# acappemin/Video-to-Audio-and-Piano-RP

Hardware: AMD Instinct MI355X
Metric: mel-frames/sec (10s VGGSound shape, 32-step CFM, CFG 2.0) (higher is better)
Workload: dtype bf16x3; 1 GPU; BASELINE.json configs[1]: 1 clip(s)/GPU x 750 latent frames x 128 ch, 32-point sway grid = 31 CFG evaluations (62 DiT forwards), T5 context 16 tokens, V2A zero roll; clips_per_gpu=1, global_clips=1, parallelism=clip-sharded x1, 1 all-gather, hipgraph=True, schedule=three streams, side_streams=True, cascade_passes=1

## Files before the change

### video-to-audio-and-piano-rp_amd/csrc/gemm_8phase.hip

```cpp
#include "gemm_common.h"

namespace {

#if defined(V2A_GEMM_PROBE) && defined(V2A_8PH_SKIP)
constexpr int kSkip = V2A_8PH_SKIP;
#else
constexpr int kSkip = 0;
#endif

template <int EPI, typename OutT, int MODE>
__global__ __launch_bounds__(512) void gemm_bf16_8ph_kernel(GemmParams p) {
  constexpr bool STAGGER = MODE != 2;
  constexpr int BM = 256, BN = 256, WM = 128, WN = 64, TM = 8, TN = 4;
  constexpr int HALF = 128 * 128;
  constexpr int BUF = 4 * HALF;
  static_assert(EPI != V2A_EPI_GEGLU || (TN % 2 == 0), "GEGLU needs value/gate tile pairs");
  extern __shared__ __attribute__((aligned(16))) char smem_raw[];

  const int tid = threadIdx.x;
  const int lane = tid & 63;
  const int wave = __builtin_amdgcn_readfirstlane(tid >> 6);
  const int wr = wave >> 2, wc = wave & 3;
  const int lr = lane & 15, lq = lane >> 4;

  int tm, tn;
  tile_of_block(p, blockIdx.x, tm, tn);
  const int m0 = tm * BM, n0 = tn * BN;

  f32x4 acc[TM][TN];
#pragma unroll
  for (int i = 0; i < TM; ++i)
#pragma unroll
    for (int j = 0; j < TN; ++j) acc[i][j] = f32x4{0.f, 0.f, 0.f, 0.f};

  const int srow = lane >> 3;
  const uint32_t schunk_b = (uint32_t)(((lane & 7) ^ srow) << 4);
  uint32_t woff[2][2];
#pragma unroll
  for (int s = 0; s < 2; ++s)
#pragma unroll
    for (int i = 0; i < 2; ++i) {
      const int r = 8 * (wave + 8 * i) + srow;
      const int wrw = n0 + 64 * (r >> 5) + (r & 31) + 32 * s;
      woff[s][i] = (uint32_t)(((int64_t)(wrw < p.N ? wrw : p.N - 1) * p.ldw) * 2) + schunk_b;
    }
  const char* wbase = reinterpret_cast<const char*>(p.w);
  const int nk = p.K / 64;

  const int nseg = p.nseg;
  const int64_t a0 = (int64_t)p.a[0];
  const int64_t da1 = nseg > 1 ? (int64_t)p.a[1] - a0 : 0, da2 = nseg > 2 ? (int64_t)p.a[2] - (int64_t)p.a[1] : 0;
  const int32_t ldb0 = (int32_t)(p.lda[0] * 2);
  const int32_t dl1 = nseg > 1 ? (int32_t)(p.lda[1] * 2) - ldb0 : 0, dl2 = nseg > 2 ? (int32_t)((p.lda[2] - p.lda[1]) * 2) : 0;
  const int kend0 = nseg > 1 ? p.kend[0] : 0x7fffffff, kend1 = nseg > 2 ? p.kend[1] : 0x7fffffff;
  const int dk2 = nseg > 2 ? p.kend[1] - p.kend[0] : 0;
  const int kl = p.s3_kl;
  const int nkl = kl > 0 ? kl / 64 : 0x3fffffff;
  const int klog = kl > 0 ? kl : p.K;
  const int sb0 = kl > 0 ? (int)(2 * p.alo[0]) : 0;
  const int dsb1 = kl > 0 && nseg > 1 ? (int)(2 * p.alo[1]) - sb0 : 0;
  const int dsb2 = kl > 0 && nseg > 2 ? (int)(2 * p.alo[2]) - (sb0 + dsb1) : 0;
  const int64_t wlo = (int64_t)kl * 2;
  const char* aptr[2];
  int aleft[2] = {0, 0};
  uint32_t aoff[2][2];
  auto a_setup = [&](int s, int kt) {
    const bool p1 = kt >= nkl, p2 = kt >= 2 * nkl;
    const int k0 = (kt - (p1 ? nkl : 0) - (p2 ? nkl : 0)) * 64;
    const bool s1 = k0 >= kend0, s2 = k0 >= kend1;
    const int kbeg = (s1 ? kend0 : 0) + (s2 ? dk2 : 0);
    const int lo = p2 ? sb0 + (s1 ? dsb1 : 0) + (s2 ? dsb2 : 0) : 0;
    aptr[s] = reinterpret_cast<const char*>(a0 + (s1 ? da1 : 0) + (s2 ? da2 : 0)) + (int64_t)(k0 - kbeg) * 2 + lo;
    const uint32_t ldb = (uint32_t)(ldb0 + (s1 ? dl1 : 0) + (s2 ? dl2 : 0));
    const int kstop = min(klog, s2 ? 0x7fffffff : (s1 ? kend1 : kend0));
    aleft[s] = (kstop - k0) >> 6;
#pragma unroll
    for (int i = 0; i < 2; ++i) {
      const int r = 8 * (wave + 8 * i) + srow;
      const int ar = m0 + r + ((r >= 64) ? 64 : 0) + 64 * s;
      aoff[s][i] = (uint32_t)(ar < p.M ? ar : p.M - 1) * ldb + schunk_b;
    }
  };
  auto stage_a = [&](int s, int kt, int buf) {
    if (aleft[s] == 0) a_setup(s, kt);
    char* dst = smem_raw + buf * BUF + s * HALF;
#pragma unroll
    for (int i = 0; i < 2; ++i)
      __builtin_amdgcn_global_load_lds((const __attribute__((address_space(1))) void*)(aptr[s] + aoff[s][i]),
                                       (__attribute__((address_space(3))) void*)(dst + (wave + 8 * i) * 1024), 16, 0, 0);
    aptr[s] += 128;
    --aleft[s];
  };
  const char* wptr = wbase;
  int wleft = 0;
  auto stage_b = [&](int kt, int buf) {
    if (wleft == 0) {
      const bool p1 = kt >= nkl, p2 = kt >= 2 * nkl;
      const int ktl = kt - (p1 ? nkl : 0) - (p2 ? nkl : 0);
      wptr = wbase + (int64_t)ktl * 128 + (p1 && !p2 ? wlo : 0);
      wleft = min(nkl, nk) - ktl;
    }
#pragma unroll
    for (int s = 0; s < 2; ++s) {
      char* dst = smem_raw + buf * BUF + (2 + s) * HALF;
#pragma unroll
      for (int i = 0; i < 2; ++i) {
        uint32_t wo = woff[s][i];
        asm volatile("" : "+v"(wo));
        __builtin_amdgcn_global_load_lds((const __attribute__((address_space(1))) void*)(wptr + wo),
                                         (__attribute__((address_space(3))) void*)(dst + (wave + 8 * i) * 1024), 16, 0, 0);
      }
    }
    wptr += 128;
    --wleft;
  };

  const int a_frag_off = (64 * wr + lr) * 128;
  const int b_frag_off = (32 * wc + lr) * 128;
  const int ch0 = ((0 + lq) ^ (lr & 7)) << 4, ch1 = ((4 + lq) ^ (lr & 7)) << 4;
  bf16x8 af[4][2], bf0[2][2], bf1[2][2];
  auto read_a = [&](int s, int buf) {
    const char* base = smem_raw + buf * BUF + s * HALF + a_frag_off;
#pragma unroll
    for (int i = 0; i < 4; ++i) {
      af[i][0] = *reinterpret_cast<const bf16x8*>(base + i * 2048 + ch0);
      af[i][1] = *reinterpret_cast<const bf16x8*>(base + i * 2048 + ch1);
    }
  };
  auto read_b = [&](int s, int buf, bf16x8 (&bf)[2][2]) {
    const char* base = smem_raw + buf * BUF + (2 + s) * HALF + b_frag_off;
#pragma unroll
    for (int j = 0; j < 2; ++j) {
      bf[j][0] = *reinterpret_cast<const bf16x8*>(base + j * 2048 + ch0);
      bf[j][1] = *reinterpret_cast<const bf16x8*>(base + j * 2048 + ch1);
    }
  };
  const int rows_valid = (p.dbg & 512) ? 256 : p.M - m0;
  const bool need0 = wr * 128 < rows_valid, need1 = wr * 128 + 64 < rows_valid;
  auto quadrant = [&](auto sa_c, auto sb_c, const bf16x8 (&bf)[2][2]) {
    constexpr int SA = decltype(sa_c)::value, SB = decltype(sb_c)::value;
    if (!(SA == 0 ? need0 : need1)) return;
    __builtin_amdgcn_s_setprio(1);
#pragma unroll
    for (int kk = 0; kk < 2; ++kk)
#pragma unroll
      for (int i = 0; i < 4; ++i)
#pragma unroll
        for (int j = 0; j < 2; ++j)
          acc[4 * SA + i][2 * SB + j] = __builtin_amdgcn_mfma_f32_16x16x32_bf16(af[i][kk], bf[j][kk], acc[4 * SA + i][2 * SB + j], 0, 0, 0);
    __builtin_amdgcn_s_setprio(0);
  };
  using I0 = std::integral_constant<int, 0>;
  using I1 = std::integral_constant<int, 1>;

  float* rs_lds = reinterpret_cast<float*>(smem_raw + 2 * BUF);
  const bool scaled = p.rssq != nullptr && p.vec_epi;
  RowScaleLoad rsl;
  if (scaled && tid < 256) rowscale_load(p, m0 + tid, rsl);
  stage_a(0, 0, 0);
  stage_b(0, 0);
  stage_a(1, 0, 0);
  if (nk > 1) {
    stage_a(0, 1, 1);
    stage_b(1, 1);
    if (scaled && tid < 256) rs_lds[tid] = rowscale_finish(p, rsl);
    asm volatile("s_waitcnt vmcnt(6)" ::: "memory");
  } else {
    if (scaled && tid < 256) rs_lds[tid] = rowscale_finish(p, rsl);
    asm volatile("s_waitcnt vmcnt(0)" ::: "memory");
  }
  __builtin_amdgcn_s_barrier();
  if constexpr (STAGGER) {
    if (wr == 1) __builtin_amdgcn_s_barrier();
  }

  auto ktile = [&](auto buf_c, int t) {
    constexpr int B = decltype(buf_c)::value;
    if (!(kSkip & 4) || t == 0) read_a(0, B);
    if (!(kSkip & 1) || t == 0) read_b(0, B, bf0);
    __builtin_amdgcn_sched_barrier(0);
    __builtin_amdgcn_s_barrier();
    quadrant(I0{}, I0{}, bf0);
    __builtin_amdgcn_sched_barrier(0);
    __builtin_amdgcn_s_barrier();
    if (!(kSkip & 1) || t == 0) read_b(1, B, bf1);
    if (t + 1 < nk && !(kSkip & 8)) stage_a(1, t + 1, B ^ 1);
    __builtin_amdgcn_sched_barrier(0);
    __builtin_amdgcn_s_barrier();
    quadrant(I0{}, I1{}, bf1);
    __builtin_amdgcn_sched_barrier(0);
    __builtin_amdgcn_s_barrier();
    if (!(kSkip & 4) || t == 0) read_a(1, B);
    if (t + 2 < nk && !(kSkip & 8)) stage_a(0, t + 2, B);
    __builtin_amdgcn_sched_barrier(0);
    __builtin_amdgcn_s_barrier();
    quadrant(I1{}, I1{}, bf1);
    __builtin_amdgcn_sched_barrier(0);
    __builtin_amdgcn_s_barrier();
    if (t + 2 < nk) {
      if (!(kSkip & 2)) stage_b(t + 2, B);
      asm volatile("s_waitcnt vmcnt(6)" ::: "memory");
    } else {
      asm volatile("s_waitcnt vmcnt(0)" ::: "memory");
    }
    __builtin_amdgcn_sched_barrier(0);
    __builtin_amdgcn_s_barrier();
    quadrant(I1{}, I0{}, bf0);
    __builtin_amdgcn_sched_barrier(0);
    __builtin_amdgcn_s_barrier();
  };
  for (int t = 0; t < nk; t += 2) {
    ktile(I0{}, t);
    if (t + 1 < nk) ktile(I1{}, t + 1);
  }
  if constexpr (STAGGER) {
    if (wr == 0) __builtin_amdgcn_s_barrier();
  }
  if (p.vec_epi) {
    static_assert(8 * 16 * (WN + 4) * 4 <= 2 * BUF, "epilogue slabs must fit in the ring memory");
    float* tile = reinterpret_cast<float*>(smem_raw) + wave * (16 * (WN + 4));
    EpiPrefetch<EPI, TM, WN, false> pf;
    gemm_epilogue_lds<EPI, OutT, TM, TN, WM, WN, false>(p, acc, tile, m0 + wr * WM, n0 + wc * WN, lane, pf, scaled ? rs_lds + wr * WM : nullptr);
  } else {
    gemm_epilogue<EPI, OutT, TM, TN, WM, WN>(p, acc, m0, n0, wr, wc, lr, lq);
  }
}

template <int EPI, typename OutT>
int launch_8ph(const GemmParams& p_in, hipStream_t s) {
  GemmParams p = p_in;
  v2a_detail::fill_tile_map(p, 256, 256);
  constexpr size_t smem = 2 * 4 * 128 * 128 + 256 * 4;
  const int tiles = ((p.M + 255) / 256) * ((p.N + 255) / 256);
  const int mode = v2a_detail::g_gemm_tuning.use_8phase;
  auto go = [&](auto kern) -> int {
    static std::atomic<uint64_t> lds_set{0};
    if (int rc = v2a_enable_lds(reinterpret_cast<const void*>(kern), smem, lds_set, "v2a_gemm(8-phase)")) return rc;
    hipLaunchKernelGGL(kern, dim3(tiles), dim3(512), smem, s, p);
    return 0;
  };
  int rc;
  if (mode == 2) rc = go(gemm_bf16_8ph_kernel<EPI, OutT, 2>);
  else rc = go(gemm_bf16_8ph_kernel<EPI, OutT, 1>);
  if (rc) return rc;
  return v2a_check_launch("v2a_gemm(8-phase)");
}

}

int v2a_detail::launch_gemm_8phase(const GemmParams& p, int epilogue, int out_dtype, hipStream_t s) {
  const bool out_f32 = out_dtype == V2A_F32;
  switch (epilogue) {
    case V2A_EPI_STORE:
      return out_f32 ? launch_8ph<V2A_EPI_STORE, float>(p, s) : launch_8ph<V2A_EPI_STORE, bf16_t>(p, s);
    case V2A_EPI_GEGLU:
      return out_f32 ? launch_8ph<V2A_EPI_GEGLU, float>(p, s) : launch_8ph<V2A_EPI_GEGLU, bf16_t>(p, s);
    case V2A_EPI_RESID:
      if (out_f32) return launch_8ph<V2A_EPI_RESID, float>(p, s);
      break;
    case V2A_EPI_GATE_RESID:
      if (out_f32) return launch_8ph<V2A_EPI_GATE_RESID, float>(p, s);
      break;
  }
  return v2a_fail(V2A_ERR_ARG, "v2a_gemm(8-phase): unsupported epilogue %d / out_dtype %d", epilogue, out_dtype);
}
```

### video-to-audio-and-piano-rp_amd/csrc/gemm_common.h

```cpp
#pragma once
#include "v2a_common.h"
#include <stdlib.h>
#include <type_traits>

namespace v2a_detail {

struct GemmParams {
  const void* a[3];
  int64_t lda[3];
  int32_t kend[3];
  int32_t nseg;
  const void* w;
  int64_t ldw;
  const float* bias;
  int32_t M, N, K;
  void* out;
  int64_t ldo;
  bf16_t* out2;
  int64_t ldo2;
  const float* resid;
  int64_t ldr;
  const float* gate;
  const int32_t* step;
  int64_t gss, gbs;
  int32_t rpb;
  const float* rope;
  int32_t rope_cols, rope_pos_off;
  int32_t vec_epi;
  int32_t relu;
  const int32_t* a_rowoff;
  const int32_t* a_koff;
  const int32_t* o_rowoff;
  int32_t krot;
  const float* ngam;
  int64_t ngss, ngbs;
  int32_t nsw_row, nsw_off;
  float* ssq;
  int64_t ssq_ld;
  const float* rssq;
  int64_t rssq_ld;
  int32_t rssq_parts;
  float rnorm;
  int32_t xcd_gm, xcd_gn;
  struct Rect { int32_t m_lo, n_lo, cnt, hm; float rcp; } rect[8];
  int32_t nrect, tiles_m, tiles_n;
  int32_t out2_split, out_split;
  int64_t alo[3];
  int64_t out2_lo;
  int32_t s3_kl;
  int32_t dbg;
};

struct GemmTuning {
  int force_tile;
  int krot;
  int use_8phase;
  int min_tiles_8phase;
  int xcd_grid;
  int dbg;
};
extern GemmTuning g_gemm_tuning;
extern int g_attn_one_group_from;
extern int g_dwconv_rows_per_wave;
extern int g_probe_dbg;
extern int g_dwconv_stream;

int launch_gemm_8phase(const GemmParams& p, int epilogue, int out_dtype, hipStream_t stream);

inline void fill_tile_map(GemmParams& p, int BM, int BN) {
  p.tiles_m = (p.M + BM - 1) / BM;
  p.tiles_n = (p.N + BN - 1) / BN;
  const int gm = p.xcd_gm, gn = p.xcd_gn;
  p.nrect = gm * gn;
  for (int r = 0; r < p.nrect; ++r) {
    const int xm = r / gn, xn = r % gn;
    const int m_lo = xm * p.tiles_m / gm, m_hi = (xm + 1) * p.tiles_m / gm;
    const int n_lo = xn * p.tiles_n / gn, n_hi = (xn + 1) * p.tiles_n / gn;
    const int hm = m_hi - m_lo;
    p.rect[r].m_lo = m_lo;
    p.rect[r].n_lo = n_lo;
    p.rect[r].cnt = hm * (n_hi - n_lo);
    p.rect[r].hm = hm > 0 ? hm : 1;
    p.rect[r].rcp = 1.0f / (float)(hm > 0 ? hm : 1);
  }
}

}

namespace {

using v2a_detail::GemmParams;

__device__ __forceinline__ void tile_of_index(const GemmParams& p, int L, int& tm, int& tn) {
  tm = tn = 0;
#pragma unroll
  for (int r = 0; r < 8; ++r) {
    if (r < p.nrect) {
      const int cnt = p.rect[r].cnt;
      if (L >= 0 && L < cnt) {
        const int hm = p.rect[r].hm;
        int q = (int)((float)L * p.rect[r].rcp);
        int rem = L - q * hm;
        if (rem < 0) { --q; rem += hm; }
        else if (rem >= hm) { ++q; rem -= hm; }
        tn = p.rect[r].n_lo + q;
        tm = p.rect[r].m_lo + rem;
      }
      L -= cnt;
    }
  }
}
__device__ __forceinline__ void tile_of_block(const GemmParams& p, int bid, int& tm, int& tn) {
  const int nwg = p.tiles_m * p.tiles_n;
  const int q = nwg >> 3, r = nwg & 7, xcd = bid & 7;
  const int L = (xcd < r ? xcd * (q + 1) : r * (q + 1) + (xcd - r) * q) + (bid >> 3);
  tile_of_index(p, L, tm, tn);
}

template <typename T> struct TileCfg;
template <> struct TileCfg<bf16_t> {
  static constexpr int BK = 64;
  static constexpr int LDS_ROW = 64;
};
template <> struct TileCfg<float> {
  static constexpr int BK = 16;
  static constexpr int LDS_ROW = 20;
};

template <int ROWS, bool SRC_F32> struct StageBf16 {
  static constexpr int N = ROWS / 32;
  bf16x8 r[N];
  __device__ __forceinline__ void load(const void* base, int64_t ld, int row0, int rows_total, int k0, int tid) {
    const int chunk = tid & 7;
#pragma unroll
    for (int i = 0; i < N; ++i) {
      int row = row0 + (tid >> 3) + 32 * i;
      row = row < rows_total ? row : rows_total - 1;
      if constexpr (SRC_F32) {
        const float* p = reinterpret_cast<const float*>(base) + (int64_t)row * ld + k0 + chunk * 8;
        f32x4 lo = *reinterpret_cast<const f32x4*>(p);
        f32x4 hi = *reinterpret_cast<const f32x4*>(p + 4);
        bf16x8 v;
#pragma unroll
        for (int j = 0; j < 4; ++j) {
          v[j] = (bf16_t)lo[j];
          v[4 + j] = (bf16_t)hi[j];
        }
        r[i] = v;
      } else {
        const bf16_t* p = reinterpret_cast<const bf16_t*>(base) + (int64_t)row * ld + k0 + chunk * 8;
        r[i] = *reinterpret_cast<const bf16x8*>(p);
      }
    }
  }
  __device__ __forceinline__ void store(bf16_t* lds, int tid) const {
    const int chunk = tid & 7;
#pragma unroll
    for (int i = 0; i < N; ++i) {
      int row = (tid >> 3) + 32 * i;
      *reinterpret_cast<bf16x8*>(lds + row * 64 + ((chunk ^ (row & 7)) << 3)) = r[i];
    }
  }
};

template <int ROWS> struct StageF32 {
  static constexpr int N = ROWS / 64;
  f32x4 r[N];
  __device__ __forceinline__ void load(const void* base, int64_t ld, int row0, int rows_total, int k0, int tid) {
    const int c4 = tid & 3;
#pragma unroll
    for (int i = 0; i < N; ++i) {
      int row = row0 + (tid >> 2) + 64 * i;
      row = row < rows_total ? row : rows_total - 1;
      const float* p = reinterpret_cast<const float*>(base) + (int64_t)row * ld + k0 + c4 * 4;
      r[i] = *reinterpret_cast<const f32x4*>(p);
    }
  }
  __device__ __forceinline__ void store(float* lds, int tid) const {
    const int c4 = tid & 3;
#pragma unroll
    for (int i = 0; i < N; ++i) {
      int row = (tid >> 2) + 64 * i;
      *reinterpret_cast<f32x4*>(lds + row * 20 + c4 * 4) = r[i];
    }
  }
};

template <typename T, bool A_F32, int ROWS> struct StageSel;
template <bool A_F32, int ROWS> struct StageSel<bf16_t, A_F32, ROWS> { using type = StageBf16<ROWS, A_F32>; };
template <bool A_F32, int ROWS> struct StageSel<float, A_F32, ROWS> { using type = StageF32<ROWS>; };

template <int EPI, typename OutT, int TM, int TN, int WM, int WN>
__device__ __forceinline__ void gemm_epilogue(const GemmParams& p, f32x4 (&acc)[TM][TN], int m0, int n0, int wm, int wn,
                                              int lr, int lq) {
  OutT* out = reinterpret_cast<OutT*>(p.out);
#pragma unroll
  for (int i = 0; i < TM; ++i) {
#pragma unroll
    for (int jj = 0; jj < 4; ++jj) {
      const int m = m0 + wm * WM + i * 16 + lq * 4 + jj;
      if (m >= p.M) continue;
      const float* gvec = nullptr;
      if constexpr (EPI == V2A_EPI_GATE_RESID) gvec = step_vec(p.gate, p.step, p.gss, p.gbs, p.gbs ? m / p.rpb : 0);
      if constexpr (EPI == V2A_EPI_GEGLU) {
#pragma unroll
        for (int j = 0; j < TN; j += 2) {
          const int n = n0 + wn * WN + j * 16 + lr;
          if (n >= p.N) continue;
          float v = acc[i][j][jj], g = acc[i][j + 1][jj];
          if (p.bias) { v += p.bias[n]; g += p.bias[n + 16]; }
          const int oc = ((n0 + wn * WN) >> 1) + (j >> 1) * 16 + lr;
          const float ge = sizeof(OutT) == 2 ? gelu_fast_f(g) : gelu_erf_f(g);
          out[(int64_t)m * p.ldo + oc] = from_f32<OutT>(v * ge);
        }
      } else {
#pragma unroll
        for (int j = 0; j < TN; ++j) {
          const int n = n0 + wn * WN + j * 16 + lr;
          if (n >= p.N) continue;
          float v = acc[i][j][jj];
          if (p.bias) v += p.bias[n];
          if constexpr (EPI == V2A_EPI_SIGMOID) v = sigmoid_f(v);
          if constexpr (EPI == V2A_EPI_RESID) v += p.resid[(int64_t)m * p.ldr + n];
          if constexpr (EPI == V2A_EPI_GATE_RESID) v = p.resid[(int64_t)m * p.ldr + n] + gvec[n] * v;
          if (p.relu) v = fmaxf(v, 0.f);
          out[(int64_t)m * p.ldo + n] = from_f32<OutT>(v);
          if constexpr (sizeof(OutT) == 4) {
            if (p.out2) p.out2[(int64_t)m * p.ldo2 + n] = (bf16_t)v;
          }
        }
      }
    }
  }
}


template <int EPI, int TM, int WN, bool ON> struct EpiPrefetch {
  static constexpr int LPR = WN / 4, RPI = 64 / LPR, RPS = 16 / RPI;
  static constexpr bool RES = ON && (EPI == V2A_EPI_RESID || EPI == V2A_EPI_GATE_RESID);
  static constexpr bool GATE = ON && EPI == V2A_EPI_GATE_RESID;
  f32x4 rs[RES ? TM : 1][RES ? RPS : 1];
  f32x4 gt[GATE ? TM : 1][GATE ? RPS : 1];
  static constexpr bool SCAT = RES && !GATE;
  int32_t ro[SCAT ? TM : 1][SCAT ? RPS : 1];
  static constexpr bool ROPE = ON && EPI == V2A_EPI_STORE;
  f32x4 cs[ROPE ? TM : 1][ROPE ? RPS : 1];
  __device__ __forceinline__ void load(const GemmParams& p, int m_base, int n_base, int lane) {
    if constexpr (ROPE) {
      const int c4 = (lane % LPR) * 4, r0 = lane / LPR;
      const int n = n_base + c4;
      if (p.rope && n < p.rope_cols) {
#pragma unroll
        for (int i = 0; i < TM; ++i)
#pragma unroll
          for (int q = 0; q < RPS; ++q) {
            int m = m_base + i * 16 + r0 + q * RPI;
            m = m < p.M ? m : p.M - 1;
            const int pos = p.rope_pos_off + m % p.rpb;
            cs[i][q] = *reinterpret_cast<const f32x4*>(p.rope + ((int64_t)pos * 32 + ((n & 63) >> 1)) * 2);
          }
      }
    }
    if constexpr (RES) {
      const int c4 = (lane % LPR) * 4, r0 = lane / LPR;
      const int n = n_base + c4;
      const int M = p.M;
      const bool full = n + 3 < p.N;
      const bool has_res = p.resid != nullptr, has_gate = p.gate != nullptr;
      const float* resid = p.resid + n;
      const int64_t ldr = p.ldr;
      const int32_t* orow = SCAT ? p.o_rowoff : nullptr;
      if constexpr (SCAT) {
        if (orow) {
#pragma unroll
          for (int i = 0; i < TM; ++i)
#pragma unroll
            for (int q = 0; q < RPS; ++q) {
              int m = m_base + i * 16 + r0 + q * RPI;
              m = m < M ? m : M - 1;
              ro[i][q] = orow[m];
            }
        }
      }
#pragma unroll
      for (int i = 0; i < TM; ++i)
#pragma unroll
        for (int q = 0; q < RPS; ++q) {
          const int m = m_base + i * 16 + r0 + q * RPI;
          if (m < M && full) {
            int64_t off = (int64_t)m * ldr;
            if constexpr (SCAT) { if (orow) off = ro[i][q]; }
            rs[i][q] = has_res ? *reinterpret_cast<const f32x4*>(resid + off) : f32x4{0.f, 0.f, 0.f, 0.f};
            if constexpr (GATE) gt[i][q] = has_gate ? *reinterpret_cast<const f32x4*>(step_vec(p.gate, p.step, p.gss, p.gbs, p.gbs ? m / p.rpb : 0) + n) : f32x4{1.f, 1.f, 1.f, 1.f};
          }
        }
    }
  }
};

constexpr int kRowSsqMax = 40;
struct RowScaleLoad {
  f32x4 v[kRowSsqMax / 4];
};
__device__ __forceinline__ void rowscale_load(const GemmParams& p, int m, RowScaleLoad& r) {
  m = m < p.M ? m : p.M - 1;
  const float* q = p.rssq + (int64_t)m * p.rssq_ld;
#pragma unroll
  for (int k = 0; k < kRowSsqMax / 4; ++k) {
    r.v[k] = f32x4{0.f, 0.f, 0.f, 0.f};
    if (4 * k < p.rssq_parts) r.v[k] = *reinterpret_cast<const f32x4*>(q + 4 * k);
  }
}
__device__ __forceinline__ float rowscale_finish(const GemmParams& p, const RowScaleLoad& r) {
  float s = 0.f;
#pragma unroll
  for (int k = 0; k < kRowSsqMax / 4; ++k) s += (r.v[k][0] + r.v[k][1]) + (r.v[k][2] + r.v[k][3]);
  return p.rnorm / fmaxf(sqrtf(s), 1e-12f);
}

template <int EPI, typename OutT, int TM, int TN, int WM, int WN, bool PF>
__device__ __forceinline__ void gemm_epilogue_lds(const GemmParams& p, f32x4 (&acc)[TM][TN], float* tile ,
                                                  int m_base, int n_base, int lane, const EpiPrefetch<EPI, TM, WN, PF>& pf,
                                                  const float* rs_row = nullptr ) {
  constexpr int LD = WN + 4;
  const int lr = lane & 15, lq = lane >> 4;
  OutT* out = reinterpret_cast<OutT*>(p.out);
  const int M = p.M;
  const bool relu = p.relu != 0;
  const int32_t* orow = p.o_rowoff;
  const int64_t ldo = p.ldo, ldr = p.ldr, ldo2 = p.ldo2;
  bf16_t* out2 = p.out2;
  const float* resid = p.resid;
  constexpr int LPRX = (EPI == V2A_EPI_GEGLU ? WN / 2 : WN) / 4;
  constexpr int RPSX = 16 / (64 / LPRX);
  f32x4 gmA = {1.f, 1.f, 1.f, 1.f}, gmB = gmA;
  if constexpr ((EPI == V2A_EPI_RESID || EPI == V2A_EPI_GATE_RESID) && sizeof(OutT) == 4) {
    const int nn = n_base + (lane % (WN / 4)) * 4;
    if (out2 && p.ngam && p.ngbs == 0 && nn + 3 < p.N) {
      const float* gb = step_vec(p.ngam, p.step, p.ngss, 0, 0) + nn;
      gmA = *reinterpret_cast<const f32x4*>(gb);
      gmB = *reinterpret_cast<const f32x4*>(gb + p.nsw_off);
    }
  }
  float rsc[TM][RPSX];
  const bool scaled = rs_row != nullptr;
  const bool geglu_wide = EPI == V2A_EPI_GEGLU && sizeof(OutT) == 2 && ((uintptr_t)p.out & 15) == 0 && (p.ldo & 7) == 0 && ((p.N >> 1) & 7) == 0 &&
                          !(p.dbg & 128);
  if (scaled) {
#pragma unroll
    for (int i = 0; i < TM; ++i)
#pragma unroll
      for (int q = 0; q < RPSX; ++q) rsc[i][q] = rs_row[i * 16 + lane / LPRX + q * (64 / LPRX)];
  }
#pragma unroll
  for (int i = 0; i < TM; ++i) {
    if (m_base + i * 16 >= M) continue;
#pragma unroll
    for (int j = 0; j < TN; ++j)
#pragma unroll
      for (int jj = 0; jj < 4; ++jj) tile[(lq * 4 + jj) * LD + j * 16 + lr] = acc[i][j][jj];
    if constexpr (EPI == V2A_EPI_GEGLU && sizeof(OutT) == 2 && (WN / 2) % 32 == 0) {
      if (geglu_wide) {
        constexpr int OC = WN / 2, LPR = OC / 8, RPI = 64 / LPR;
        static_assert(RPI <= 16, "one slab holds 16 rows");
        const int c8 = (lane % LPR) * 8, r0 = lane / LPR;
        const int lc = (c8 >> 4) * 32 + (c8 & 15);
        const int n = n_base + lc;
        f32x4 bv[2] = {{0.f, 0.f, 0.f, 0.f}, {0.f, 0.f, 0.f, 0.f}}, bg[2] = {{0.f, 0.f, 0.f, 0.f}, {0.f, 0.f, 0.f, 0.f}};
        if (p.bias && n < p.N) {
          bv[0] = *reinterpret_cast<const f32x4*>(p.bias + n);
          bv[1] = *reinterpret_cast<const f32x4*>(p.bias + n + 4);
          bg[0] = *reinterpret_cast<const f32x4*>(p.bias + n + 16);
          bg[1] = *reinterpret_cast<const f32x4*>(p.bias + n + 20);
        }
#pragma unroll
        for (int q = 0; q < 16 / RPI; ++q) {
          const int r = r0 + q * RPI;
          const int m = m_base + i * 16 + r;
          if (m >= p.M || n >= p.N) continue;
          const float rs = scaled ? rs_row[i * 16 + r] : 1.f;
          bf16x8 hi, lo;
#pragma unroll
          for (int h2 = 0; h2 < 2; ++h2) {
            f32x4 v = *reinterpret_cast<const f32x4*>(tile + r * LD + lc + 4 * h2);
            f32x4 g = *reinterpret_cast<const f32x4*>(tile + r * LD + lc + 16 + 4 * h2);
            if (scaled) {
              v *= rs;
              g *= rs;
            }
#pragma unroll
            for (int e = 0; e < 4; ++e) {
              const float o32 = (v[e] + bv[h2][e]) * gelu_fast_f(g[e] + bg[h2][e]);
              hi[4 * h2 + e] = (bf16_t)o32;
              lo[4 * h2 + e] = (bf16_t)(o32 - (float)hi[4 * h2 + e]);
            }
          }
          OutT* dst = out + (int64_t)m * p.ldo + (n_base >> 1) + c8;
          *reinterpret_cast<bf16x8*>(dst) = hi;
          if (p.out_split) *reinterpret_cast<bf16x8*>(dst + (p.N >> 1)) = lo;
        }
        continue;
      }
    }
    if constexpr (EPI == V2A_EPI_GEGLU) {
      constexpr int OC = WN / 2;
      constexpr int LPR = OC / 4;
      constexpr int RPI = 64 / LPR;
      const int c4 = (lane % LPR) * 4, r0 = lane / LPR;
      const int lc = (c4 >> 4) * 32 + (c4 & 15);
      const int n = n_base + lc;
      f32x4 bv = {0.f, 0.f, 0.f, 0.f}, bg = {0.f, 0.f, 0.f, 0.f};
      if (p.bias && n < p.N) {
        bv = *reinterpret_cast<const f32x4*>(p.bias + n);
        bg = *reinterpret_cast<const f32x4*>(p.bias + n + 16);
      }
#pragma unroll
      for (int q = 0; q < 16 / RPI; ++q) {
        const int r = r0 + q * RPI;
        const int m = m_base + i * 16 + r;
        if (m >= p.M || n >= p.N) continue;
        f32x4 v = *reinterpret_cast<const f32x4*>(tile + r * LD + lc);
        f32x4 g = *reinterpret_cast<const f32x4*>(tile + r * LD + lc + 16);
        if (scaled) {
          v *= rsc[i][q];
          g *= rsc[i][q];
        }
        OutT* dst = out + (int64_t)m * p.ldo + (n_base >> 1) + c4;
        if constexpr (sizeof(OutT) == 2) {
          if (p.out_split) {
            bf16x4 hi, lo;
#pragma unroll
            for (int e = 0; e < 4; ++e) {
              const float o32 = (v[e] + bv[e]) * gelu_fast_f(g[e] + bg[e]);
              hi[e] = (bf16_t)o32;
              lo[e] = (bf16_t)(o32 - (float)hi[e]);
            }
            *reinterpret_cast<bf16x4*>(dst) = hi;
            *reinterpret_cast<bf16x4*>(dst + (p.N >> 1)) = lo;
          } else {
            bf16x4 o;
#pragma unroll
            for (int e = 0; e < 4; ++e) o[e] = (bf16_t)((v[e] + bv[e]) * gelu_fast_f(g[e] + bg[e]));
            *reinterpret_cast<bf16x4*>(dst) = o;
          }
        } else {
          f32x4 o;
#pragma unroll
          for (int e = 0; e < 4; ++e) o[e] = (v[e] + bv[e]) * gelu_erf_f(g[e] + bg[e]);
          *reinterpret_cast<f32x4*>(dst) = o;
        }
      }
    } else {
      constexpr int LPR = WN / 4;
      constexpr int RPI = 64 / LPR;
      const int c4 = (lane % LPR) * 4, r0 = lane / LPR;
      const int n = n_base + c4;
      const bool full = n + 3 < p.N;
      f32x4 bv = {0.f, 0.f, 0.f, 0.f};
      if (p.bias && full) bv = *reinterpret_cast<const f32x4*>(p.bias + n);
#pragma unroll
      for (int q = 0; q < 16 / RPI; ++q) {
        const int r = r0 + q * RPI;
        const int m = m_base + i * 16 + r;
        if (m >= M || !full) continue;
        int64_t o_out = (int64_t)m * ldo, o_res = (int64_t)m * ldr, o_out2 = (int64_t)m * ldo2;
        if constexpr (EPI == V2A_EPI_STORE || EPI == V2A_EPI_RESID) {
          if (orow) {
            int64_t ro;
            if constexpr (PF && EPI == V2A_EPI_RESID) ro = pf.ro[i][q];
            else ro = orow[m];
            o_out = o_res = o_out2 = ro;
          }
        }
        f32x4 v = *reinterpret_cast<const f32x4*>(tile + r * LD + c4);
        if (scaled) v *= rsc[i][q];
#pragma unroll
        for (int e = 0; e < 4; ++e) v[e] += bv[e];
        if constexpr (EPI == V2A_EPI_SIGMOID) {
#pragma unroll
          for (int e = 0; e < 4; ++e) v[e] = sigmoid_f(v[e]);
        }
        if constexpr (EPI == V2A_EPI_STORE) {
          if (p.rope && n < p.rope_cols) {
            f32x4 cs;
            if constexpr (PF) cs = pf.cs[i][q];
            else cs = *reinterpret_cast<const f32x4*>(p.rope + ((int64_t)(p.rope_pos_off + m % p.rpb) * 32 + ((n & 63) >> 1)) * 2);
            const float a0 = v[0], b0 = v[1], a1 = v[2], b1 = v[3];
            v[0] = fmaf(a0, cs[0], -(b0 * cs[1]));
            v[1] = fmaf(b0, cs[0], a0 * cs[1]);
            v[2] = fmaf(a1, cs[2], -(b1 * cs[3]));
            v[3] = fmaf(b1, cs[2], a1 * cs[3]);
          }
        }
        if constexpr (EPI == V2A_EPI_RESID || EPI == V2A_EPI_GATE_RESID) {
          f32x4 rs, gt = {1.f, 1.f, 1.f, 1.f};
          if constexpr (PF) {
            rs = pf.rs[i][q];
            if constexpr (EPI == V2A_EPI_GATE_RESID) gt = pf.gt[i][q];
          } else {
            rs = resid ? *reinterpret_cast<const f32x4*>(resid + o_res + n) : f32x4{0.f, 0.f, 0.f, 0.f};
            if constexpr (EPI == V2A_EPI_GATE_RESID) {
              if (p.gate) gt = *reinterpret_cast<const f32x4*>(step_vec(p.gate, p.step, p.gss, p.gbs, p.gbs ? m / p.rpb : 0) + n);
            }
          }
#pragma unroll
          for (int e = 0; e < 4; ++e) v[e] = rs[e] + gt[e] * v[e];
        }
        if (relu) {
#pragma unroll
          for (int e = 0; e < 4; ++e) v[e] = fmaxf(v[e], 0.f);
        }
        if constexpr (sizeof(OutT) == 2) {
          bf16x4 o;
#pragma unroll
          for (int e = 0; e < 4; ++e) o[e] = (bf16_t)v[e];
          *reinterpret_cast<bf16x4*>(out + o_out + n) = o;
        } else {
          *reinterpret_cast<f32x4*>(out + o_out + n) = v;
          if (out2) {
            f32x4 gm = m >= p.nsw_row ? gmB : gmA;
            if (p.ngam && p.ngbs) gm = *reinterpret_cast<const f32x4*>(step_vec(p.ngam, p.step, p.ngss, p.ngbs, m / p.rpb) + (m >= p.nsw_row ? p.nsw_off : 0) + n);
            bf16x4 o;
#pragma unroll
            for (int e = 0; e < 4; ++e) o[e] = (bf16_t)(v[e] * gm[e]);
            *reinterpret_cast<bf16x4*>(out2 + o_out2 + n) = o;
            if (p.out2_split) {
              bf16x4 lo;
#pragma unroll
              for (int e = 0; e < 4; ++e) lo[e] = (bf16_t)(v[e] * gm[e] - (float)o[e]);
              *reinterpret_cast<bf16x4*>(out2 + o_out2 + p.out2_lo + n) = lo;
            }
            if (p.ssq) {
              const float ss = octet_sum(v[0] * v[0] + v[1] * v[1] + v[2] * v[2] + v[3] * v[3]);
              if ((lane & 7) == 0) p.ssq[(int64_t)m * p.ssq_ld + (n >> 5)] = ss;
            }
          }
        }
      }
    }
  }
}

}
```

Measured before the change: 3176 mel-frames/s.

## Software-pipeline GEMM epilogue loads and hoist bias/step lookups out of row loops

Restructures the LDS-staged GEMM epilogue so residual and RoPE operands for the next 16-row slab are fetched while the current slab is processed. Bias vectors, the step index and the invariant gate/gamma vectors are loaded once per wave instead of per row. Interior slabs get an unguarded fast path, and row scales are computed per slab on the non-prefetch path to save registers. The 8-phase kernel also drops the row-offset indirection at compile time. This trades extra live registers and hand-placed vmcnt waits for less global-load latency in the epilogue.

```diff
diff --git a/video-to-audio-and-piano-rp_amd/csrc/gemm_8phase.hip b/video-to-audio-and-piano-rp_amd/csrc/gemm_8phase.hip
--- a/video-to-audio-and-piano-rp_amd/csrc/gemm_8phase.hip
+++ b/video-to-audio-and-piano-rp_amd/csrc/gemm_8phase.hip
@@ -220,7 +220,7 @@
     static_assert(8 * 16 * (WN + 4) * 4 <= 2 * BUF, "epilogue slabs must fit in the ring memory");
     float* tile = reinterpret_cast<float*>(smem_raw) + wave * (16 * (WN + 4));
     EpiPrefetch<EPI, TM, WN, false> pf;
-    gemm_epilogue_lds<EPI, OutT, TM, TN, WM, WN, false>(p, acc, tile, m0 + wr * WM, n0 + wc * WN, lane, pf, scaled ? rs_lds + wr * WM : nullptr);
+    gemm_epilogue_lds<EPI, OutT, TM, TN, WM, WN, false, false>(p, acc, tile, m0 + wr * WM, n0 + wc * WN, lane, pf, scaled ? rs_lds + wr * WM : nullptr);
   } else {
     gemm_epilogue<EPI, OutT, TM, TN, WM, WN>(p, acc, m0, n0, wr, wc, lr, lq);
   }
diff --git a/video-to-audio-and-piano-rp_amd/csrc/gemm_common.h b/video-to-audio-and-piano-rp_amd/csrc/gemm_common.h
--- a/video-to-audio-and-piano-rp_amd/csrc/gemm_common.h
+++ b/video-to-audio-and-piano-rp_amd/csrc/gemm_common.h
@@ -194,6 +194,14 @@
 __device__ __forceinline__ void gemm_epilogue(const GemmParams& p, f32x4 (&acc)[TM][TN], int m0, int n0, int wm, int wn,
                                               int lr, int lq) {
   OutT* out = reinterpret_cast<OutT*>(p.out);
+  const int64_t step = EPI == V2A_EPI_GATE_RESID && p.step ? (int64_t)p.step[0] : 0;
+  float bcol[TN];
+#pragma unroll
+  for (int j = 0; j < TN; ++j) {
+    const int n = n0 + wn * WN + j * 16 + lr;
+    const int nb = EPI == V2A_EPI_GEGLU ? n - 16 * (j & 1) : n;
+    bcol[j] = p.bias && nb < p.N ? p.bias[n] : 0.f;
+  }
 #pragma unroll
   for (int i = 0; i < TM; ++i) {
 #pragma unroll
@@ -201,14 +209,14 @@
       const int m = m0 + wm * WM + i * 16 + lq * 4 + jj;
       if (m >= p.M) continue;
       const float* gvec = nullptr;
-      if constexpr (EPI == V2A_EPI_GATE_RESID) gvec = step_vec(p.gate, p.step, p.gss, p.gbs, p.gbs ? m / p.rpb : 0);
+      if constexpr (EPI == V2A_EPI_GATE_RESID) gvec = p.gate + step * p.gss + (p.gbs ? (int64_t)(m / p.rpb) * p.gbs : 0);
       if constexpr (EPI == V2A_EPI_GEGLU) {
 #pragma unroll
         for (int j = 0; j < TN; j += 2) {
           const int n = n0 + wn * WN + j * 16 + lr;
           if (n >= p.N) continue;
           float v = acc[i][j][jj], g = acc[i][j + 1][jj];
-          if (p.bias) { v += p.bias[n]; g += p.bias[n + 16]; }
+          if (p.bias) { v += bcol[j]; g += bcol[j + 1]; }
           const int oc = ((n0 + wn * WN) >> 1) + (j >> 1) * 16 + lr;
           const float ge = sizeof(OutT) == 2 ? gelu_fast_f(g) : gelu_erf_f(g);
           out[(int64_t)m * p.ldo + oc] = from_f32<OutT>(v * ge);
@@ -219,7 +227,7 @@
           const int n = n0 + wn * WN + j * 16 + lr;
           if (n >= p.N) continue;
           float v = acc[i][j][jj];
-          if (p.bias) v += p.bias[n];
+          if (p.bias) v += bcol[j];
           if constexpr (EPI == V2A_EPI_SIGMOID) v = sigmoid_f(v);
           if constexpr (EPI == V2A_EPI_RESID) v += p.resid[(int64_t)m * p.ldr + n];
           if constexpr (EPI == V2A_EPI_GATE_RESID) v = p.resid[(int64_t)m * p.ldr + n] + gvec[n] * v;
@@ -318,7 +326,9 @@
   return p.rnorm / fmaxf(sqrtf(s), 1e-12f);
 }
 
-template <int EPI, typename OutT, int TM, int TN, int WM, int WN, bool PF>
+constexpr int kVmcnt0 = 0x0f70;
+
+template <int EPI, typename OutT, int TM, int TN, int WM, int WN, bool PF, bool ROWOFF = true>
 __device__ __forceinline__ void gemm_epilogue_lds(const GemmParams& p, f32x4 (&acc)[TM][TN], float* tile ,
                                                   int m_base, int n_base, int lane, const EpiPrefetch<EPI, TM, WN, PF>& pf,
                                                   const float* rs_row = nullptr ) {
@@ -327,34 +337,94 @@
   OutT* out = reinterpret_cast<OutT*>(p.out);
   const int M = p.M;
   const bool relu = p.relu != 0;
-  const int32_t* orow = p.o_rowoff;
+  const int32_t* orow = ROWOFF ? p.o_rowoff : nullptr;
   const int64_t ldo = p.ldo, ldr = p.ldr, ldo2 = p.ldo2;
   bf16_t* out2 = p.out2;
   const float* resid = p.resid;
   constexpr int LPRX = (EPI == V2A_EPI_GEGLU ? WN / 2 : WN) / 4;
   constexpr int RPSX = 16 / (64 / LPRX);
+  const int64_t step = p.step ? (int64_t)p.step[0] : 0;
   f32x4 gmA = {1.f, 1.f, 1.f, 1.f}, gmB = gmA;
   if constexpr ((EPI == V2A_EPI_RESID || EPI == V2A_EPI_GATE_RESID) && sizeof(OutT) == 4) {
     const int nn = n_base + (lane % (WN / 4)) * 4;
     if (out2 && p.ngam && p.ngbs == 0 && nn + 3 < p.N) {
-      const float* gb = step_vec(p.ngam, p.step, p.ngss, 0, 0) + nn;
+      const float* gb = p.ngam + step * p.ngss + nn;
       gmA = *reinterpret_cast<const f32x4*>(gb);
       gmB = *reinterpret_cast<const f32x4*>(gb + p.nsw_off);
     }
   }
-  float rsc[TM][RPSX];
   const bool scaled = rs_row != nullptr;
+  float rsc[PF ? TM : 1][RPSX];
+  auto row_scales = [&](int i) {
+    if (scaled) {
+#pragma unroll
+      for (int q = 0; q < RPSX; ++q) rsc[PF ? i : 0][q] = rs_row[i * 16 + lane / LPRX + q * (64 / LPRX)];
+    }
+  };
   const bool geglu_wide = EPI == V2A_EPI_GEGLU && sizeof(OutT) == 2 && ((uintptr_t)p.out & 15) == 0 && (p.ldo & 7) == 0 && ((p.N >> 1) & 7) == 0 &&
                           !(p.dbg & 128);
-  if (scaled) {
-#pragma unroll
-    for (int i = 0; i < TM; ++i)
-#pragma unroll
-      for (int q = 0; q < RPSX; ++q) rsc[i][q] = rs_row[i * 16 + lane / LPRX + q * (64 / LPRX)];
-  }
-#pragma unroll
-  for (int i = 0; i < TM; ++i) {
-    if (m_base + i * 16 >= M) continue;
+  if constexpr (PF) {
+#pragma unroll
+    for (int i = 0; i < TM; ++i) row_scales(i);
+  }
+  constexpr int LPRG = WN / 4, RPIG = 64 / LPRG, RPSG = 16 / RPIG;
+  const int g_c4 = (lane % LPRG) * 4, g_r0 = lane / LPRG, g_n = n_base + g_c4;
+  const bool g_full = g_n + 3 < p.N;
+  f32x4 gbv[2] = {{0.f, 0.f, 0.f, 0.f}, {0.f, 0.f, 0.f, 0.f}}, gbg[2] = {{0.f, 0.f, 0.f, 0.f}, {0.f, 0.f, 0.f, 0.f}};
+  if constexpr (EPI != V2A_EPI_GEGLU) {
+    if (p.bias && g_full) gbv[0] = *reinterpret_cast<const f32x4*>(p.bias + g_n);
+  } else {
+    const bool wide = sizeof(OutT) == 2 && (WN / 2) % 32 == 0 && geglu_wide;
+    const int c = wide ? (lane % (WN / 16)) * 8 : (lane % (WN / 8)) * 4;
+    const int n = n_base + (c >> 4) * 32 + (c & 15);
+    if (p.bias && n < p.N) {
+      gbv[0] = *reinterpret_cast<const f32x4*>(p.bias + n);
+      gbg[0] = *reinterpret_cast<const f32x4*>(p.bias + n + 16);
+      if (wide) {
+        gbv[1] = *reinterpret_cast<const f32x4*>(p.bias + n + 4);
+        gbg[1] = *reinterpret_cast<const f32x4*>(p.bias + n + 20);
+      }
+    }
+  }
+  constexpr bool AHEAD = !PF && EPI != V2A_EPI_GEGLU && EPI != V2A_EPI_SIGMOID;
+  constexpr bool A_ROPE = AHEAD && EPI == V2A_EPI_STORE;
+  constexpr bool A_RES = AHEAD && (EPI == V2A_EPI_RESID || EPI == V2A_EPI_GATE_RESID);
+  constexpr bool A_GATE = AHEAD && EPI == V2A_EPI_GATE_RESID;
+  struct SlabOps {
+    f32x4 cs[A_ROPE ? RPSG : 1];
+    f32x4 rs[A_RES ? RPSG : 1];
+  };
+  SlabOps cur, nxt;
+  f32x4 gt_inv = {1.f, 1.f, 1.f, 1.f};
+  const float* gate_n = nullptr;
+  if constexpr (A_GATE) {
+    if (p.gate && g_full) {
+      gate_n = p.gate + step * p.gss + g_n;
+      if (p.gbs == 0) gt_inv = *reinterpret_cast<const f32x4*>(gate_n);
+    }
+  }
+  auto fetch = [&](int i, SlabOps& o) {
+    if constexpr (AHEAD) {
+      const bool rope_on = A_ROPE && p.rope && g_n < p.rope_cols;
+#pragma unroll
+      for (int q = 0; q < RPSG; ++q) {
+        const int m = m_base + i * 16 + g_r0 + q * RPIG;
+        if (m >= M || !g_full) continue;
+        if constexpr (A_ROPE) {
+          if (rope_on) o.cs[q] = *reinterpret_cast<const f32x4*>(p.rope + ((int64_t)(p.rope_pos_off + m % p.rpb) * 32 + ((g_n & 63) >> 1)) * 2);
+        }
+        if constexpr (A_RES) {
+          int64_t o_res = (int64_t)m * ldr;
+          if constexpr (EPI == V2A_EPI_RESID) { if (orow) o_res = orow[m]; }
+          o.rs[q] = resid ? *reinterpret_cast<const f32x4*>(resid + o_res + g_n) : f32x4{0.f, 0.f, 0.f, 0.f};
+        }
+      }
+    }
+  };
+  fetch(0, cur);
+  if constexpr (!PF) __builtin_amdgcn_s_waitcnt(kVmcnt0);
+  auto slab = [&](int i, auto guard_c) {
+    constexpr bool GUARD = decltype(guard_c)::value;
 #pragma unroll
     for (int j = 0; j < TN; ++j)
 #pragma unroll
@@ -366,18 +436,12 @@
         const int c8 = (lane % LPR) * 8, r0 = lane / LPR;
         const int lc = (c8 >> 4) * 32 + (c8 & 15);
         const int n = n_base + lc;
-        f32x4 bv[2] = {{0.f, 0.f, 0.f, 0.f}, {0.f, 0.f, 0.f, 0.f}}, bg[2] = {{0.f, 0.f, 0.f, 0.f}, {0.f, 0.f, 0.f, 0.f}};
-        if (p.bias && n < p.N) {
-          bv[0] = *reinterpret_cast<const f32x4*>(p.bias + n);
-          bv[1] = *reinterpret_cast<const f32x4*>(p.bias + n + 4);
-          bg[0] = *reinterpret_cast<const f32x4*>(p.bias + n + 16);
-          bg[1] = *reinterpret_cast<const f32x4*>(p.bias + n + 20);
-        }
+        const f32x4 (&bv)[2] = gbv, (&bg)[2] = gbg;
 #pragma unroll
         for (int q = 0; q < 16 / RPI; ++q) {
           const int r = r0 + q * RPI;
           const int m = m_base + i * 16 + r;
-          if (m >= p.M || n >= p.N) continue;
+          if (GUARD && (m >= p.M || n >= p.N)) continue;
           const float rs = scaled ? rs_row[i * 16 + r] : 1.f;
           bf16x8 hi, lo;
 #pragma unroll
@@ -399,7 +463,7 @@
           *reinterpret_cast<bf16x8*>(dst) = hi;
           if (p.out_split) *reinterpret_cast<bf16x8*>(dst + (p.N >> 1)) = lo;
         }
-        continue;
+        return;
       }
     }
     if constexpr (EPI == V2A_EPI_GEGLU) {
@@ -409,21 +473,17 @@
       const int c4 = (lane % LPR) * 4, r0 = lane / LPR;
       const int lc = (c4 >> 4) * 32 + (c4 & 15);
       const int n = n_base + lc;
-      f32x4 bv = {0.f, 0.f, 0.f, 0.f}, bg = {0.f, 0.f, 0.f, 0.f};
-      if (p.bias && n < p.N) {
-        bv = *reinterpret_cast<const f32x4*>(p.bias + n);
-        bg = *reinterpret_cast<const f32x4*>(p.bias + n + 16);
-      }
+      const f32x4 bv = gbv[0], bg = gbg[0];
 #pragma unroll
       for (int q = 0; q < 16 / RPI; ++q) {
         const int r = r0 + q * RPI;
         const int m = m_base + i * 16 + r;
-        if (m >= p.M || n >= p.N) continue;
+        if (GUARD && (m >= p.M || n >= p.N)) continue;
         f32x4 v = *reinterpret_cast<const f32x4*>(tile + r * LD + lc);
         f32x4 g = *reinterpret_cast<const f32x4*>(tile + r * LD + lc + 16);
         if (scaled) {
-          v *= rsc[i][q];
-          g *= rsc[i][q];
+          v *= rsc[PF ? i : 0][q];
+          g *= rsc[PF ? i : 0][q];
         }
         OutT* dst = out + (int64_t)m * p.ldo + (n_base >> 1) + c4;
         if constexpr (sizeof(OutT) == 2) {
@@ -456,13 +516,12 @@
       const int c4 = (lane % LPR) * 4, r0 = lane / LPR;
       const int n = n_base + c4;
       const bool full = n + 3 < p.N;
-      f32x4 bv = {0.f, 0.f, 0.f, 0.f};
-      if (p.bias && full) bv = *reinterpret_cast<const f32x4*>(p.bias + n);
+      const f32x4 bv = gbv[0];
 #pragma unroll
       for (int q = 0; q < 16 / RPI; ++q) {
         const int r = r0 + q * RPI;
         const int m = m_base + i * 16 + r;
-        if (m >= M || !full) continue;
+        if (GUARD && (m >= M || !full)) continue;
         int64_t o_out = (int64_t)m * ldo, o_res = (int64_t)m * ldr, o_out2 = (int64_t)m * ldo2;
         if constexpr (EPI == V2A_EPI_STORE || EPI == V2A_EPI_RESID) {
           if (orow) {
@@ -473,7 +532,7 @@
           }
         }
         f32x4 v = *reinterpret_cast<const f32x4*>(tile + r * LD + c4);
-        if (scaled) v *= rsc[i][q];
+        if (scaled) v *= rsc[PF ? i : 0][q];
 #pragma unroll
         for (int e = 0; e < 4; ++e) v[e] += bv[e];
         if constexpr (EPI == V2A_EPI_SIGMOID) {
@@ -484,7 +543,7 @@
           if (p.rope && n < p.rope_cols) {
             f32x4 cs;
             if constexpr (PF) cs = pf.cs[i][q];
-            else cs = *reinterpret_cast<const f32x4*>(p.rope + ((int64_t)(p.rope_pos_off + m % p.rpb) * 32 + ((n & 63) >> 1)) * 2);
+            else cs = cur.cs[q];
             const float a0 = v[0], b0 = v[1], a1 = v[2], b1 = v[3];
             v[0] = fmaf(a0, cs[0], -(b0 * cs[1]));
             v[1] = fmaf(b0, cs[0], a0 * cs[1]);
@@ -498,9 +557,10 @@
             rs = pf.rs[i][q];
             if constexpr (EPI == V2A_EPI_GATE_RESID) gt = pf.gt[i][q];
           } else {
-            rs = resid ? *reinterpret_cast<const f32x4*>(resid + o_res + n) : f32x4{0.f, 0.f, 0.f, 0.f};
+            rs = cur.rs[q];
             if constexpr (EPI == V2A_EPI_GATE_RESID) {
-              if (p.gate) gt = *reinterpret_cast<const f32x4*>(step_vec(p.gate, p.step, p.gss, p.gbs, p.gbs ? m / p.rpb : 0) + n);
+              gt = gt_inv;
+              if (gate_n && p.gbs) gt = *reinterpret_cast<const f32x4*>(gate_n + (int64_t)(m / p.rpb) * p.gbs);
             }
           }
 #pragma unroll
@@ -519,7 +579,7 @@
           *reinterpret_cast<f32x4*>(out + o_out + n) = v;
           if (out2) {
             f32x4 gm = m >= p.nsw_row ? gmB : gmA;
-            if (p.ngam && p.ngbs) gm = *reinterpret_cast<const f32x4*>(step_vec(p.ngam, p.step, p.ngss, p.ngbs, m / p.rpb) + (m >= p.nsw_row ? p.nsw_off : 0) + n);
+            if (p.ngam && p.ngbs) gm = *reinterpret_cast<const f32x4*>(p.ngam + step * p.ngss + (int64_t)(m / p.rpb) * p.ngbs + (m >= p.nsw_row ? p.nsw_off : 0) + n);
             bf16x4 o;
 #pragma unroll
             for (int e = 0; e < 4; ++e) o[e] = (bf16_t)(v[e] * gm[e]);
@@ -538,7 +598,20 @@
         }
       }
     }
-  }
-}
-
-}
+  };
+#pragma unroll
+  for (int i = 0; i < TM; ++i) {
+    if (m_base + i * 16 >= M) break;
+    if (i + 1 < TM) fetch(i + 1, nxt);
+    if constexpr (!PF) row_scales(i);
+    if (!PF && m_base + i * 16 + 16 <= M && n_base + WN <= p.N) {
+      slab(i, std::false_type{});
+    } else {
+      slab(i, std::true_type{});
+      if constexpr (!PF) __builtin_amdgcn_s_waitcnt(kVmcnt0);
+    }
+    if constexpr (AHEAD) cur = nxt;
+  }
+}
+
+}
```

New measurement: 3205 mel-frames/s (median of 6 runs). No clear change (+0.9%).
